# siyi-wind/MDViT

Measured on AMD Instinct MI355X. Metric: 512x512 images/sec MDViT train step (fwd+bwd, two-sweep, AdamW), higher is better.
Workload: dtype bf16x3 (fp32 storage; GEMM operands split hi+lo bf16, fp32 accumulate); 1 GPU; MDViT Sup+MLPFM train step, 4 domain(s) x bs=4 per GPU, 512x512, drop_rate=0.1 drop_path=0.1, bf16x3 GEMMs, data-parallel x1

## Files before the change

mdvit_amd/csrc/attn.hip:

```cpp
#include "common.h"
#include "conv_tile.h"

namespace {

constexpr int FA_T = 64;

struct FaGeom {
    int B, H, W, N, C, heads, Ch, s3, s5, s7;
    float scale;
};

typedef float fap_f32x16 __attribute__((ext_vector_type(16)));

template <int CH, bool SOFTMAX>
__global__ __launch_bounds__(256) void fa_partial_kernel(const float* __restrict__ X, long ldx, const float* __restrict__ Y, long ldy,
                                                         const float* __restrict__ ysc, float yscale,
                                                         float* __restrict__ ws_m, float* __restrict__ ws_s, float* __restrict__ ws_P,
                                                         FaGeom g, int NT, int NSUB,
                                                         const float* __restrict__ outp = nullptr, float* __restrict__ dU = nullptr, float* __restrict__ e_part = nullptr) {
    constexpr int GW = CH < 32 ? 32 : CH, NB = (GW + 31) / 32, GQ = GW / 4;
    constexpr int STAGE = 2 * FA_T * GW, RED = 4 * NB * 32 * NB * 32;
    __shared__ __attribute__((aligned(16))) float sm[(STAGE > RED ? STAGE : RED) + 3 * NB * 32 + (SOFTMAX ? 2 * 256 : 0)];
    float* xs = sm;
    float* ys = sm + FA_T * GW;
    float* s_m = sm + (STAGE > RED ? STAGE : RED);
    float* s_s = s_m + NB * 32;
    float* s_f = s_s + NB * 32;
    float* s_e = s_s;
    float* s_pm = s_f + NB * 32;
    float* s_ps = s_pm + 256;
    const int stile = blockIdx.x, c0 = blockIdx.y * GW, b = blockIdx.z;
    const int NTS = (NT + NSUB - 1) / NSUB;
    const int lane = threadIdx.x & 63, wave = threadIdx.x >> 6, l31 = lane & 31, lhi = lane >> 5;
    fap_f32x16 acc[NB][NB];
#pragma unroll
    for (int i = 0; i < NB; ++i)
#pragma unroll
        for (int j = 0; j < NB; ++j)
#pragma unroll
            for (int r = 0; r < 16; ++r) acc[i][j][r] = 0.f;
    if (SOFTMAX && threadIdx.x < NB * 32) { s_m[threadIdx.x] = -INFINITY; s_s[threadIdx.x] = 0.f; s_f[threadIdx.x] = 1.f; }
    if (SOFTMAX) s_ps[threadIdx.x] = 0.f;
    if (!SOFTMAX && e_part && threadIdx.x < NB * 32) s_e[threadIdx.x] = 0.f;
    constexpr int NVE = (FA_T * GQ + 255) / 256;
    float4 eacc[(!SOFTMAX) ? NVE : 1];
#pragma unroll
    for (int v = 0; v < ((!SOFTMAX) ? NVE : 1); ++v) eacc[v] = make_float4(0.f, 0.f, 0.f, 0.f);
    constexpr int NV = (FA_T * GQ + 255) / 256;
    float4 xv[NV], yv[NV], ov[(!SOFTMAX) ? NV : 1];
    auto request = [&](int tile) __attribute__((always_inline)) {
        const int n0r = min(tile, NT - 1) * FA_T;
#pragma unroll
        for (int v = 0; v < NV; ++v) {
            const int i = min((int)threadIdx.x + 256 * v, FA_T * GQ - 1), n = i / GQ, q = i % GQ;
            const long tok = (long)b * g.N + min(n0r + n, g.N - 1);
            xv[v] = *reinterpret_cast<const float4*>(X + tok * ldx + c0 + 4 * q);
            yv[v] = *reinterpret_cast<const float4*>(Y + tok * ldy + c0 + 4 * q);
            if (!SOFTMAX && e_part) ov[v] = *reinterpret_cast<const float4*>(outp + tok * (long)g.C + c0 + 4 * q);
        }
    };
    request(stile * NSUB);
    for (int sub = 0; sub < NSUB; ++sub) {
        const int tile = stile * NSUB + sub;
        if (tile >= NT) break;
        const int n0 = tile * FA_T, nt = min(FA_T, g.N - n0);
        {
#pragma unroll
            for (int v = 0; v < NV; ++v) {
                const int i = threadIdx.x + 256 * v, n = i / GQ;
                if (!(i < FA_T * GQ && n < nt)) {
                    xv[v] = make_float4(0.f, 0.f, 0.f, 0.f); yv[v] = xv[v];
                    if (!SOFTMAX) ov[v] = xv[v];
                }
            }
#pragma unroll
            for (int v = 0; v < NV; ++v) {
                const int i = threadIdx.x + 256 * v, n = i / GQ, q = i % GQ;
                if (i < FA_T * GQ) {
                    float4 y4 = yv[v];
                    if (!SOFTMAX) {
                        float4 sc = make_float4(yscale, yscale, yscale, yscale);
                        float4 a4 = make_float4(1.f, 1.f, 1.f, 1.f);
                        if (ysc) { a4 = *reinterpret_cast<const float4*>(ysc + (long)b * g.C + c0 + 4 * q); sc.x *= a4.x; sc.y *= a4.y; sc.z *= a4.z; sc.w *= a4.w; }
                        if (dU && n < nt)
                            *reinterpret_cast<float4*>(dU + ((long)b * g.N + n0 + n) * g.C + c0 + 4 * q) =
                                make_float4(a4.x * y4.x * xv[v].x, a4.y * y4.y * xv[v].y, a4.z * y4.z * xv[v].z, a4.w * y4.w * xv[v].w);
                        if (e_part) {
                            eacc[v].x = fmaf(y4.x, ov[v].x, eacc[v].x); eacc[v].y = fmaf(y4.y, ov[v].y, eacc[v].y);
                            eacc[v].z = fmaf(y4.z, ov[v].z, eacc[v].z); eacc[v].w = fmaf(y4.w, ov[v].w, eacc[v].w);
                        }
                        y4.x *= sc.x; y4.y *= sc.y; y4.z *= sc.z; y4.w *= sc.w;
                    }
                    *reinterpret_cast<float4*>(xs + n * GW + 4 * q) = xv[v];
                    *reinterpret_cast<float4*>(ys + n * GW + 4 * q) = y4;
                }
            }
        }
        if (sub + 1 < NSUB) request(tile + 1);
        __syncthreads();
        if (SOFTMAX) {
            constexpr int PER = 256 / GW;
            const int c = threadIdx.x % GW, sb = threadIdx.x / GW;
            const bool act = sb < PER;
            float m = -INFINITY;
            if (act)
                for (int n = sb; n < nt; n += PER) m = fmaxf(m, xs[n * GW + c]);
            if (act) s_pm[sb * GW + c] = m;
            __syncthreads();
            float m_old = 0.f, m_new = 0.f;
            if (act) {
                m_old = s_m[c];
                m_new = m_old;
#pragma unroll
                for (int j = 0; j < PER; ++j) m_new = fmaxf(m_new, s_pm[j * GW + c]);
                float ssum = 0.f;
                for (int n = sb; n < nt; n += PER) { const float e = expf(xs[n * GW + c] - m_new); xs[n * GW + c] = e; ssum += e; }
                for (int n = nt + sb; n < FA_T; n += PER) xs[n * GW + c] = 0.f;
                const float f = expf(m_old - m_new);
                s_ps[sb * GW + c] = fmaf(s_ps[sb * GW + c], f, ssum);
                if (sb == 0) s_f[c] = f;
            }
            __syncthreads();
            if (act && sb == 0) s_m[c] = m_new;
            if (sub > 0) {
#pragma unroll
                for (int i = 0; i < NB; ++i)
#pragma unroll
                    for (int q = 0; q < 4; ++q) {
                        const float4 f4 = *reinterpret_cast<const float4*>(s_f + 32 * i + 8 * q + 4 * lhi);
#pragma unroll
                        for (int j = 0; j < NB; ++j) {
                            acc[i][j][4 * q + 0] *= f4.x; acc[i][j][4 * q + 1] *= f4.y; acc[i][j][4 * q + 2] *= f4.z; acc[i][j][4 * q + 3] *= f4.w;
                        }
                    }
            }
        }
        constexpr int TPW = FA_T / 4;
#pragma unroll
        for (int kk = 0; kk < TPW / 2; ++kk) {
            const int n = wave * TPW + 2 * kk + lhi;
            float xa[NB], yb[NB];
#pragma unroll
            for (int i = 0; i < NB; ++i) { const int c = 32 * i + l31; xa[i] = c < GW ? xs[n * GW + c] : 0.f; }
#pragma unroll
            for (int j = 0; j < NB; ++j) { const int c = 32 * j + l31; yb[j] = c < GW ? ys[n * GW + c] : 0.f; }
#pragma unroll
            for (int i = 0; i < NB; ++i)
#pragma unroll
                for (int j = 0; j < NB; ++j) acc[i][j] = __builtin_amdgcn_mfma_f32_32x32x2f32(xa[i], yb[j], acc[i][j], 0, 0, 0);
        }
        __syncthreads();
    }
    if (SOFTMAX && threadIdx.x < GW) {
        const long o = ((long)b * NTS + stile) * g.C + c0 + threadIdx.x;
        float ssum = 0.f;
#pragma unroll
        for (int j = 0; j < 256 / GW; ++j) ssum += s_ps[j * GW + threadIdx.x];
        ws_m[o] = s_m[threadIdx.x]; ws_s[o] = ssum;
    }
    if (!SOFTMAX && e_part) {
#pragma unroll
        for (int v = 0; v < NVE; ++v) {
            const int i = threadIdx.x + 256 * v, q = i % GQ;
            if (i < FA_T * GQ) {
                atomicAdd(&s_e[4 * q + 0], eacc[v].x); atomicAdd(&s_e[4 * q + 1], eacc[v].y);
                atomicAdd(&s_e[4 * q + 2], eacc[v].z); atomicAdd(&s_e[4 * q + 3], eacc[v].w);
            }
        }
        __syncthreads();
        if (threadIdx.x < GW) e_part[((long)b * NTS + stile) * g.C + c0 + threadIdx.x] = s_e[threadIdx.x];
        __syncthreads();
    }
    constexpr int RW = NB * 32;
    float* red = sm + wave * RW * RW;
#pragma unroll
    for (int i = 0; i < NB; ++i)
#pragma unroll
        for (int j = 0; j < NB; ++j)
#pragma unroll
            for (int r = 0; r < 16; ++r) {
                const int c = 32 * i + 8 * (r >> 2) + 4 * lhi + (r & 3), e = 32 * j + l31;
                red[c * RW + e] = acc[i][j][r];
            }
    __syncthreads();
    for (int o = threadIdx.x; o < GW * CH; o += 256) {
        const int c = o / CH, el = o % CH, e = (c / CH) * CH + el;
        const float v = (sm[c * RW + e] + sm[RW * RW + c * RW + e]) + (sm[2 * RW * RW + c * RW + e] + sm[3 * RW * RW + c * RW + e]);
        ws_P[(((long)b * NTS + stile) * g.C + c0 + c) * CH + el] = v;
    }
}

template <int P> __device__ __forceinline__ float fa_dpp_quad_xor(float x) {
    constexpr int ctrl = P == 1 ? 0xB1 : (P == 2 ? 0x4E : 0x1B);
    return __builtin_bit_cast(float, __builtin_amdgcn_update_dpp(0, __builtin_bit_cast(int, x), ctrl, 0xF, 0xF, true));
}
template <int CH, bool SOFTMAX>
__global__ __launch_bounds__(256) __attribute__((amdgpu_waves_per_eu(2, 2))) void fa_partial_s8_kernel(const float* __restrict__ X, long ldx, const float* __restrict__ Y, long ldy,
                                                            const float* __restrict__ ysc, float yscale,
                                                            float* __restrict__ ws_m, float* __restrict__ ws_s, float* __restrict__ ws_P,
                                                            FaGeom g, int NT, int NSUB,
                                                            const float* __restrict__ outp, float* __restrict__ dU, float* __restrict__ e_part) {
    constexpr int C = 8 * CH, LPT = C / 4, SLOTS = 256 / LPT, LPH = CH / 4;
    constexpr int NACC = 4 * CH + 8;
    constexpr int GRP = (SOFTMAX && CH == 8) ? 4 : 2;
    extern __shared__ float fa_s_red[];
    const int stile = blockIdx.x, b = blockIdx.z;
    const int NTS = (NT + NSUB - 1) / NSUB;
    const int q = threadIdx.x % LPT, slot = threadIdx.x / LPT;
    const int c0 = 4 * q, hl = q % LPH;
    const int n_beg = stile * NSUB * FA_T, n_end = min(g.N, n_beg + NSUB * FA_T);
    float acc[4][CH];
#pragma unroll
    for (int j = 0; j < 4; ++j)
#pragma unroll
        for (int l = 0; l < CH; ++l) acc[j][l] = 0.f;
    float m[4] = {-INFINITY, -INFINITY, -INFINITY, -INFINITY}, ssum[4] = {0.f, 0.f, 0.f, 0.f}, eacc[4] = {0.f, 0.f, 0.f, 0.f};
    float sc[4] = {yscale, yscale, yscale, yscale}, av[4] = {1.f, 1.f, 1.f, 1.f};
    if (!SOFTMAX && ysc) {
        const float4 a4 = *reinterpret_cast<const float4*>(ysc + (long)b * C + c0);
        av[0] = a4.x; av[1] = a4.y; av[2] = a4.z; av[3] = a4.w;
#pragma unroll
        for (int j = 0; j < 4; ++j) sc[j] *= av[j];
    }
    struct Rows { float4 x[GRP], y[GRP], o[(!SOFTMAX) ? GRP : 1]; };
    auto request = [&](Rows& r, int n0) __attribute__((always_inline)) {
#pragma unroll
        for (int u = 0; u < GRP; ++u) {
            const long tok = (long)b * g.N + min(n0 + SLOTS * u, g.N - 1);
            r.x[u] = *reinterpret_cast<const float4*>(X + tok * ldx + c0);
            r.y[u] = *reinterpret_cast<const float4*>(Y + tok * ldy + c0);
            if (!SOFTMAX && e_part) r.o[u] = *reinterpret_cast<const float4*>(outp + tok * (long)C + c0);
        }
    };
    auto compute = [&](const Rows& r, int n0) __attribute__((always_inline)) {
        float xv[GRP][4], yv[GRP][4];
        bool ok[GRP];
#pragma unroll
        for (int u = 0; u < GRP; ++u) {
            ok[u] = n0 + SLOTS * u < n_end;
            xv[u][0] = r.x[u].x; xv[u][1] = r.x[u].y; xv[u][2] = r.x[u].z; xv[u][3] = r.x[u].w;
            yv[u][0] = r.y[u].x; yv[u][1] = r.y[u].y; yv[u][2] = r.y[u].z; yv[u][3] = r.y[u].w;
        }
        if (SOFTMAX) {
            float mn[4], f[4];
#pragma unroll
            for (int j = 0; j < 4; ++j) {
                mn[j] = m[j];
#pragma unroll
                for (int u = 0; u < GRP; ++u) mn[j] = fmaxf(mn[j], ok[u] ? xv[u][j] : -INFINITY);
                f[j] = (mn[j] == -INFINITY) ? 1.f : expf(m[j] - mn[j]);
                m[j] = mn[j];
                ssum[j] *= f[j];
#pragma unroll
                for (int l = 0; l < CH; ++l) acc[j][l] *= f[j];
            }
#pragma unroll
            for (int u = 0; u < GRP; ++u)
#pragma unroll
                for (int j = 0; j < 4; ++j) { xv[u][j] = ok[u] ? expf(xv[u][j] - mn[j]) : 0.f; ssum[j] += xv[u][j]; }
        }
#pragma unroll
        for (int u = 0; u < GRP; ++u) {
            float yh[CH];
            if (!SOFTMAX) {
                if (dU && ok[u]) {
                    const long tok = (long)b * g.N + n0 + SLOTS * u;
                    *reinterpret_cast<float4*>(dU + tok * C + c0) = make_float4(av[0] * yv[u][0] * xv[u][0], av[1] * yv[u][1] * xv[u][1], av[2] * yv[u][2] * xv[u][2], av[3] * yv[u][3] * xv[u][3]);
                }
                if (e_part && ok[u]) {
                    eacc[0] = fmaf(yv[u][0], r.o[u].x, eacc[0]); eacc[1] = fmaf(yv[u][1], r.o[u].y, eacc[1]);
                    eacc[2] = fmaf(yv[u][2], r.o[u].z, eacc[2]); eacc[3] = fmaf(yv[u][3], r.o[u].w, eacc[3]);
                }
#pragma unroll
                for (int j = 0; j < 4; ++j) { yh[j] = ok[u] ? yv[u][j] * sc[j] : 0.f; }
            } else {
#pragma unroll
                for (int j = 0; j < 4; ++j) yh[j] = yv[u][j];
            }
#pragma unroll
            for (int j = 0; j < 4; ++j) {
                yh[4 + j] = fa_dpp_quad_xor<1>(yh[j]);
                if (CH == 16) { yh[8 + j] = fa_dpp_quad_xor<2>(yh[j]); yh[12 + j] = fa_dpp_quad_xor<3>(yh[j]); }
            }
#pragma unroll
            for (int j = 0; j < 4; ++j)
#pragma unroll
                for (int l = 0; l < CH; ++l) acc[j][l] = fmaf(xv[u][j], yh[l], acc[j][l]);
        }
    };
    Rows ra, rb;
    int n = n_beg + slot;
    request(ra, n);
    for (; n < n_end; n += 2 * SLOTS * GRP) {
        request(rb, n + SLOTS * GRP);
        compute(ra, n);
        request(ra, n + 2 * SLOTS * GRP);
        compute(rb, n + SLOTS * GRP);
    }
    float* mine = fa_s_red + ((long)slot * LPT + q) * (NACC + 1);
#pragma unroll
    for (int j = 0; j < 4; ++j) {
#pragma unroll
        for (int l = 0; l < CH; ++l) mine[CH * j + l] = acc[j][l];
        mine[4 * CH + j] = SOFTMAX ? m[j] : eacc[j];
        mine[4 * CH + 4 + j] = ssum[j];
    }
    __syncthreads();
    if (threadIdx.x < C) {
        const int qq = threadIdx.x >> 2, j = threadIdx.x & 3, c = 4 * qq + j;
        const int hq = qq % LPH;
        float tot[CH], t1 = 0.f, mm = -INFINITY;
#pragma unroll
        for (int l = 0; l < CH; ++l) tot[l] = 0.f;
        if (SOFTMAX) {
            for (int sl = 0; sl < SLOTS; ++sl) mm = fmaxf(mm, fa_s_red[((long)sl * LPT + qq) * (NACC + 1) + 4 * CH + j]);
        }
        for (int sl = 0; sl < SLOTS; ++sl) {
            const float* r = fa_s_red + ((long)sl * LPT + qq) * (NACC + 1);
            float f = 1.f;
            if (SOFTMAX) { const float ms = r[4 * CH + j]; f = (ms == -INFINITY) ? 0.f : expf(ms - mm); t1 = fmaf(r[4 * CH + 4 + j], f, t1); }
            else t1 += r[4 * CH + j];
#pragma unroll
            for (int l = 0; l < CH; ++l) tot[l] = SOFTMAX ? fmaf(r[CH * j + l], f, tot[l]) : tot[l] + r[CH * j + l];
        }
        const long orow = ((long)b * NTS + stile) * C + c;
        float* P = ws_P + orow * CH;
#pragma unroll
        for (int l = 0; l < CH; ++l) P[4 * (hq ^ (l >> 2)) + (l & 3)] = tot[l];
        if (SOFTMAX) { ws_m[orow] = mm; ws_s[orow] = t1; }
        else if (e_part) e_part[orow] = t1;
    }
}
template <int CH, bool SOFTMAX>
static void fa_partial_stream_launch(dim3 grid, hipStream_t s, const float* X, long ldx, const float* Y, long ldy, const float* ysc, float yscale, float* ws_m, float* ws_s,
                                     float* ws_P, const FaGeom& g, int NT, int NSUB, const float* outp, float* dU, float* e_part) {
    constexpr int C = 8 * CH, LPT = C / 4, SLOTS = 256 / LPT;
    constexpr int smem = SLOTS * LPT * (4 * CH + 8 + 1) * (int)sizeof(float);
    static bool attr[64] = {false};
    int dev = 0;
    if (hipGetDevice(&dev) != hipSuccess || dev < 0 || dev >= 64) dev = 0;
    if (!attr[dev] && smem > 48 * 1024) {
// ... 473 lines not shown
        const float v = scale * (e[(long)b * C + c] - a[(long)b * C + c] * tot);
        dz[c] = v;
        dzbuf[(long)b * C + c] = v;
    }
    __syncthreads();
    float* tpart = sm + C;
    const int BD = blockDim.x;
    const int nseg = hid <= BD ? BD / hid : 1;
    for (int i0 = 0; i0 < hid; i0 += BD) {
        const int i = i0 + (int)threadIdx.x % (hid <= BD ? hid : BD), seg = hid <= BD ? (int)threadIdx.x / hid : 0;
        if (i < hid && seg < nseg) {
            const int c_beg = (int)((long)C * seg / nseg), c_end = (int)((long)C * (seg + 1) / nseg);
            float t = 0.f;
#pragma unroll 4
            for (int c = c_beg; c < c_end; ++c) t = fmaf(dz[c], W2[(long)c * hid + i], t);
            tpart[seg * hid + i] = t;
        }
    }
    __syncthreads();
    for (int i = threadIdx.x; i < hid; i += blockDim.x) {
        float s = 0.f;
        for (int d = 0; d < D; ++d) s = fmaf(label[(long)b * D + d], W1[(long)i * D + d], s);
        const float h = s + b1[i];
        float t = 0.f;
        for (int seg = 0; seg < nseg; ++seg) t += tpart[seg * hid + i];
        hbuf[(long)b * hid + i] = fmaxf(h, 0.f);
        dhbuf[(long)b * hid + i] = h > 0.f ? t : 0.f;
    }
}
__global__ __launch_bounds__(1024) void da_bwd_stage1_kernel(const float* __restrict__ label, const float* __restrict__ W1, const float* __restrict__ b1,
                                                            const float* __restrict__ W2, const float* __restrict__ a, const float* __restrict__ e,
                                                            float* __restrict__ dzbuf, float* __restrict__ hbuf, float* __restrict__ dhbuf,
                                                            int D, int hid, int C, int heads, float scale) {
    extern __shared__ float sm[];
    da_bwd_stage1_body(sm, label, W1, b1, W2, a, e, dzbuf, hbuf, dhbuf, D, hid, C, heads, scale);
}
__device__ __forceinline__ void da_bwd_stage2_body(const float* __restrict__ label, const float* __restrict__ dzbuf,
                                                   const float* __restrict__ hbuf, const float* __restrict__ dhbuf,
                                                   float* __restrict__ dW1, float* __restrict__ db1, float* __restrict__ dW2, float* __restrict__ db2,
                                                   int B, int D, int hid, int C) {
    const long i = (long)blockIdx.x * blockDim.x + threadIdx.x;
    const long nW2 = (long)C * hid, nW1 = (long)hid * D;
    if (i < nW2) {
        const int c = (int)(i / hid), j = (int)(i % hid);
        float s = 0.f;
        for (int b = 0; b < B; ++b) s = fmaf(dzbuf[(long)b * C + c], hbuf[(long)b * hid + j], s);
        dW2[i] = s;
    } else if (i < nW2 + nW1) {
        const long k = i - nW2;
        const int j = (int)(k / D), d = (int)(k % D);
        float s = 0.f;
        for (int b = 0; b < B; ++b) s = fmaf(dhbuf[(long)b * hid + j], label[(long)b * D + d], s);
        dW1[k] = s;
    } else if (i < nW2 + nW1 + C) {
        const int c = (int)(i - nW2 - nW1);
        float s = 0.f;
        for (int b = 0; b < B; ++b) s += dzbuf[(long)b * C + c];
        db2[c] = s;
    } else if (i < nW2 + nW1 + C + hid) {
        const int j = (int)(i - nW2 - nW1 - C);
        float s = 0.f;
        for (int b = 0; b < B; ++b) s += dhbuf[(long)b * hid + j];
        db1[j] = s;
    }
}
__global__ __launch_bounds__(256) void da_bwd_stage2_kernel(const float* __restrict__ label, const float* __restrict__ dzbuf,
                                                            const float* __restrict__ hbuf, const float* __restrict__ dhbuf,
                                                            float* __restrict__ dW1, float* __restrict__ db1, float* __restrict__ dW2, float* __restrict__ db2,
                                                            int B, int D, int hid, int C) {
    da_bwd_stage2_body(label, dzbuf, hbuf, dhbuf, dW1, db1, dW2, db2, B, D, hid, C);
}
__device__ __forceinline__ long da_many_ws_offset(const MdvitDaMany& m, int i, int B) {
    long off = 0;
    for (int j = 0; j < i; ++j) off += (long)B * m.C[j] + 2L * B * m.hid[j];
    return off;
}
__global__ __launch_bounds__(1024) void da_bwd_many_stage1_kernel(MdvitDaMany m, MdvitDaManyGrads g, const float* __restrict__ label, float* __restrict__ ws, int B, int D,
                                                                 float scale) {
    extern __shared__ float sm[];
    const int i = blockIdx.y;
    if (!g.e[i]) return;
    float* dzbuf = ws + da_many_ws_offset(m, i, B);
    float* hbuf = dzbuf + (long)B * m.C[i];
    float* dhbuf = hbuf + (long)B * m.hid[i];
    da_bwd_stage1_body(sm, label, m.W1[i], m.b1[i], m.W2[i], m.a[i], g.e[i], dzbuf, hbuf, dhbuf, D, m.hid[i], m.C[i], m.heads[i], scale);
}
__global__ __launch_bounds__(256) void da_bwd_many_stage2_kernel(MdvitDaMany m, MdvitDaManyGrads g, const float* __restrict__ label, const float* __restrict__ ws, int B, int D) {
    const int i = blockIdx.y;
    const int hid = m.hid[i], C = m.C[i];
    if (!g.e[i] || (long)blockIdx.x * blockDim.x >= (long)C * hid + (long)hid * D + C + hid) return;
    const float* dzbuf = ws + da_many_ws_offset(m, i, B);
    const float* hbuf = dzbuf + (long)B * C;
    const float* dhbuf = hbuf + (long)B * hid;
    da_bwd_stage2_body(label, dzbuf, hbuf, dhbuf, g.dW1[i], g.db1[i], g.dW2[i], g.db2[i], B, D, hid, C);
}

bool make_geom(FaGeom& g, int B, int H, int W, int C, int heads, int s3, int s5, int s7) {
    if (B <= 0 || H <= 0 || W <= 0 || C <= 0 || heads <= 0 || C % heads != 0 || C % 4 != 0) return false;
    if (s3 + s5 + s7 != heads) return false;
    g.B = B; g.H = H; g.W = W; g.N = H * W; g.C = C; g.heads = heads; g.Ch = C / heads; g.s3 = s3; g.s5 = s5; g.s7 = s7;
    g.scale = 1.0f / sqrtf((float)g.Ch);
    return true;
}

size_t fa_ws_floats(int B, int N, int C, int heads) {
    const int Ch = C / heads;
    const long NT = (N + FA_T - 1) / FA_T;
    const long fwd = (long)B * NT * C * (2 + Ch);
    const long wg_rows = (long)(cdiv(C, 32) + 2) * B > 1024 ? (long)(cdiv(C, 32) + 2) * B : 1024;
    const long part = wg_rows * 32 * 50 > 1024L * B * C ? wg_rows * 32 * 50 : 1024L * B * C;
    const long bwd = 2L * B * N * C + (long)B * C * (1 + Ch) + (long)B * NT * C * Ch + part;
    return (size_t)(fwd > bwd ? fwd : bwd);
}

int fa_nsub(int NT) { return NT >= 128 ? 8 : (NT >= 64 ? 4 : (NT >= 16 ? 2 : 1)); }

bool fa_built(const FaGeom& g) { return ((g.Ch == 8 || g.Ch == 16) && g.heads == 8) || ((g.Ch == 40 || g.Ch == 64) && g.C <= 512); }
#define FA_CHECK_BUILT(fn, g) MDVIT_CHECK_ARG(fa_built(g), MDVIT_E_SHAPE, fn ": C=%d with %d heads (head dim %d) not built: built are 8 heads at C = 64 / 128 (head dim 8 / 16) " \
                                              "and head dim 40 / 64 with C <= 512 (8 heads at C = 320 / 512)", (g).C, (g).heads, (g).Ch)

int quad_grid(long work_quads, int QC, int max_blocks) {
    int a = QC, b = 256;
    while (b) { int t = a % b; a = b; b = t; }
    const int gmul = QC / a;
    long want = (work_quads + 256L * 4 - 1) / (256L * 4);
    if (want > max_blocks) want = max_blocks;
    if (want < 1) want = 1;
    return (int)((want + gmul - 1) / gmul * gmul);
}

}

extern "C" size_t mdvit_factoratt_ws_bytes(int32_t B, int32_t N, int32_t C, int32_t heads) {
    if (B <= 0 || N <= 0 || C <= 0 || heads <= 0 || C % heads) return 0;
    return fa_ws_floats(B, N, C, heads) * sizeof(float);
}

extern "C" int mdvit_factoratt_fwd(const float* qkv, const float* w3, const float* b3, const float* w5, const float* b5,
                                   const float* w7, const float* b7, const float* a, float* out, float* U, float* kmax, float* ksum, float* Mmat,
                                   void* ws, size_t ws_bytes, int32_t B, int32_t H, int32_t W, int32_t C, int32_t heads,
                                   int32_t s3, int32_t s5, int32_t s7, void* stream) {
    hipStream_t s = (hipStream_t)stream;
    FaGeom g;
    MDVIT_CHECK_ARG(make_geom(g, B, H, W, C, heads, s3, s5, s7), MDVIT_E_SHAPE, "factoratt_fwd: bad geometry B=%d H=%d W=%d C=%d heads=%d splits=%d/%d/%d", B, H, W, C, heads, s3, s5, s7);
    FA_CHECK_BUILT("factoratt_fwd", g);
    MDVIT_CHECK_ARG(ws_bytes >= fa_ws_floats(B, g.N, C, heads) * sizeof(float), MDVIT_E_WORKSPACE, "factoratt_fwd: workspace too small (%zu bytes)", ws_bytes);
    const int Ch = g.Ch, NT0 = cdiv(g.N, FA_T);
    const int NSUB = fa_nsub(NT0);
    const int NT = cdiv(NT0, NSUB);
    float* ws_m = (float*)ws;
    float* ws_s = ws_m + (long)B * NT * C;
    float* ws_P = ws_s + (long)B * NT * C;
#define FA_PART_STREAM(CHV) fa_partial_stream_launch<CHV, true>(dim3(NT, 1, B), s, qkv + C, (long)3 * C, qkv + 2 * C, (long)3 * C, nullptr, 1.f, ws_m, ws_s, ws_P, g, NT0, NSUB, nullptr, nullptr, nullptr)
#define FA_PART_TILES(CHV) hipLaunchKernelGGL((fa_partial_kernel<CHV, true>), dim3(NT, C / CHV, B), dim3(256), 0, s, \
                       qkv + C, (long)3 * C, qkv + 2 * C, (long)3 * C, (const float*)nullptr, 1.f, ws_m, ws_s, ws_P, g, NT0, NSUB)
    switch (Ch) {
        case 8: FA_PART_STREAM(8); break;
        case 16: FA_PART_STREAM(16); break;
        case 40: FA_PART_TILES(40); break;
        case 64: FA_PART_TILES(64); break;
    }
#undef FA_PART_STREAM
#undef FA_PART_TILES
    if (NT > 8)
        hipLaunchKernelGGL((fa_combine_softmax_kernel<32>), dim3(cdiv((long)C * g.Ch, 8), B), dim3(256), 0, s, ws_m, ws_s, ws_P, kmax, ksum, Mmat, g, NT);
    else if (NT > 2)
        hipLaunchKernelGGL((fa_combine_softmax_kernel<4>), dim3(cdiv((long)C * g.Ch, 64), B), dim3(256), 0, s, ws_m, ws_s, ws_P, kmax, ksum, Mmat, g, NT);
    else
        hipLaunchKernelGGL((fa_combine_softmax_kernel<1>), dim3(cdiv((long)C * g.Ch, 256), B), dim3(256), 0, s, ws_m, ws_s, ws_P, kmax, ksum, Mmat, g, NT);
    const int c5 = s3 * Ch, c7 = (s3 + s5) * Ch;
    const CtGeom cg{B, g.H, g.W};
    {
        const int xoff[3] = {2 * C, 2 * C + c5, 2 * C + c7}, yoff[3] = {0, c5, c7}, ncls[3] = {s3 * Ch, s5 * Ch, s7 * Ch};
        const float* const ws3[3] = {w3, w5, w7};
        const float* const bs3[3] = {b3, b5, b7};
        launch_conv3<false>(qkv, 3L * C, xoff, ws3, bs3, U, (long)C, yoff, cg, ncls, s);
    }
    {
        const int TLN = max(1, 256 / C), block = TLN * C;
        int tpb = TLN * 32;
        while (tpb > TLN * 8 && (long)cdiv(g.N, tpb) * B < 1024) tpb /= 2;
        while ((long)cdiv(g.N, tpb) * B > 8192) tpb *= 2;
        dim3 grid(cdiv(g.N, tpb), B);
#define FA_OUT_LAUNCH(CHV) hipLaunchKernelGGL((fa_out_kernel<CHV>), grid, dim3(block), sizeof(float) * FA_OUT_U * TLN * C, s, qkv, U, Mmat, a, out, g, TLN, tpb)
        switch (Ch) {
            case 8: FA_OUT_LAUNCH(8); break;
            case 16: FA_OUT_LAUNCH(16); break;
            case 40: FA_OUT_LAUNCH(40); break;
            case 64: FA_OUT_LAUNCH(64); break;
        }
#undef FA_OUT_LAUNCH
    }
    MDVIT_LAUNCH_CHECK();
    return MDVIT_OK;
}

extern "C" int mdvit_factoratt_bwd(const float* dout, const float* qkv, const float* out, const float* U,
                                   const float* w3, const float* b3, const float* w5, const float* b5, const float* w7, const float* b7,
                                   const float* a, const float* kmax, const float* ksum, const float* Mmat,
                                   float* dqkv, float* e, float* dw3, float* db3, float* dw5, float* db5, float* dw7, float* db7,
                                   void* ws, size_t ws_bytes, int32_t B, int32_t H, int32_t W, int32_t C, int32_t heads,
                                   int32_t s3, int32_t s5, int32_t s7, void* stream) {
    hipStream_t s = (hipStream_t)stream;
    FaGeom g;
    MDVIT_CHECK_ARG(make_geom(g, B, H, W, C, heads, s3, s5, s7), MDVIT_E_SHAPE, "factoratt_bwd: bad geometry B=%d H=%d W=%d C=%d heads=%d", B, H, W, C, heads);
    FA_CHECK_BUILT("factoratt_bwd", g);
    MDVIT_CHECK_ARG(ws_bytes >= fa_ws_floats(B, g.N, C, heads) * sizeof(float), MDVIT_E_WORKSPACE, "factoratt_bwd: workspace too small (%zu bytes)", ws_bytes);
    MDVIT_CHECK_ARG((a == nullptr) == (e == nullptr), MDVIT_E_SHAPE, "factoratt_bwd: a and e must both be given or both be NULL");
    const int Ch = g.Ch, NT = cdiv(g.N, FA_T);
    float* dU = (float*)ws;
    float* dVc = dU + (long)B * g.N * C;
    float* tcol = dVc + (long)B * g.N * C;
    float* dM = tcol + (long)B * C;
    float* ws_P = dM + (long)B * C * Ch;
    const bool want_wgrad = dw3 != nullptr;
    MDVIT_CHECK_ARG(want_wgrad ? (db3 && dw5 && db5 && dw7 && db7) : !(db3 || dw5 || db5 || dw7 || db7), MDVIT_E_SHAPE,
                    "factoratt_bwd: the six crpe gradient outputs must be all given or all NULL");
    if (dqkv == nullptr) {
        MDVIT_CHECK_ARG(e != nullptr && !want_wgrad, MDVIT_E_SHAPE, "factoratt_bwd: dqkv == NULL asks for e alone");
        const int QC0 = C / 4;
        const int gx = quad_grid((long)g.N * QC0, QC0, 512);
        float* e_part = ws_P + (long)B * NT * C * Ch;
        hipLaunchKernelGGL(fa_bwd_prep_kernel, dim3(gx, B), dim3(256), sizeof(float) * C, s, dout, qkv, out, a, (float*)nullptr, e_part, g);
        MDVIT_LAUNCH_CHECK();
        return mdvit_reduce_partials_batched(e_part, B, gx, C, e, s);
    }
    const int NSUBb = fa_nsub(NT), NTS = cdiv(NT, NSUBb);
    float* e_part = ws_P + (long)B * NT * C * Ch;
#define FA_PART_STREAM(CHV) fa_partial_stream_launch<CHV, false>(dim3(NTS, 1, B), s, qkv, (long)3 * C, dout, (long)C, a, g.scale, nullptr, nullptr, ws_P, g, NT, NSUBb, out, dU, e ? e_part : nullptr)
#define FA_PART_TILES(CHV) hipLaunchKernelGGL((fa_partial_kernel<CHV, false>), dim3(NTS, C / CHV, B), dim3(256), 0, s, \
                       qkv, (long)3 * C, dout, (long)C, a, g.scale, (float*)nullptr, (float*)nullptr, ws_P, g, NT, NSUBb, out, dU, e ? e_part : (float*)nullptr)
    switch (Ch) {
        case 8: FA_PART_STREAM(8); break;
        case 16: FA_PART_STREAM(16); break;
        case 40: FA_PART_TILES(40); break;
        case 64: FA_PART_TILES(64); break;
    }
#undef FA_PART_STREAM
#undef FA_PART_TILES
    if (e) {
        const int rc = mdvit_reduce_partials_batched(e_part, B, NTS, C, e, s);
        if (rc != MDVIT_OK) return rc;
    }
    const int c5 = s3 * Ch, c7 = (s3 + s5) * Ch;
    const CtGeom cg{B, g.H, g.W};
    if (want_wgrad) {
        float* wg_part = ws_P + (long)B * NT * C * Ch;
        const int goff[3] = {0, c5, c7}, xoff3[3] = {2 * C, 2 * C + c5, 2 * C + c7}, ncls3[3] = {s3 * Ch, s5 * Ch, s7 * Ch};
        float* const dws[3] = {dw3, dw5, dw7};
        float* const dbs[3] = {db3, db5, db7};
        launch_conv3_wgrad(dU, (long)C, goff, qkv, 3L * C, xoff3, dws, dbs, wg_part, cg, ncls3, s, 0);
    }
    {
        const int off[3] = {0, c5, c7}, ncls[3] = {s3 * Ch, s5 * Ch, s7 * Ch};
        const float* const ws3[3] = {w3, w5, w7};
        launch_conv3<true>(dU, (long)C, off, ws3, nullptr, dVc, (long)C, off, cg, ncls, s);
    }
    if (Ch >= 32) {
        const int ntiles = cdiv(g.N, 32);
        int tpb = 8;
        while (tpb > 2 && (long)cdiv(ntiles, tpb) * heads * B < 256) tpb /= 2;
        const int gx = cdiv(ntiles, tpb);
        const long nwg = (long)gx * heads * B;
        const int xcd_map = nwg % 8 == 0 && nwg < (1L << 30);
        dim3 grid = xcd_map ? dim3((unsigned)nwg, 1, 1) : dim3(gx, heads, B);
        if (Ch == 40) hipLaunchKernelGGL((fa_bwd_apply3_kernel<40>), grid, dim3(384), 0, s, dout, qkv, U, dVc, Mmat, a, kmax, ksum, ws_P, NTS, dqkv, g, tpb, gx, xcd_map);
        else hipLaunchKernelGGL((fa_bwd_apply3_kernel<64>), grid, dim3(384), 0, s, dout, qkv, U, dVc, Mmat, a, kmax, ksum, ws_P, NTS, dqkv, g, tpb, gx, xcd_map);
    } else {
        int tpbk = Ch == 8 ? 1024 : 512;
        while (tpbk > 128 && (long)cdiv(g.N, tpbk) * B < 512) tpbk /= 2;
        const dim3 grid(cdiv(g.N, tpbk), B);
        if (Ch == 8) hipLaunchKernelGGL(fa_bwd_apply_tab_kernel<8>, grid, dim3(256), 0, s, dout, qkv, U, dVc, Mmat, a, kmax, ksum, ws_P, NTS, dqkv, g, tpbk);
        else hipLaunchKernelGGL(fa_bwd_apply_tab_kernel<16>, grid, dim3(256), 0, s, dout, qkv, U, dVc, Mmat, a, kmax, ksum, ws_P, NTS, dqkv, g, tpbk);
    }
    MDVIT_LAUNCH_CHECK();
    return MDVIT_OK;
}

extern "C" int mdvit_factoratt_wgrad(const float* qkv, void* ws, size_t ws_bytes, float* dw3, float* db3, float* dw5, float* db5,
                                     float* dw7, float* db7, int32_t B, int32_t H, int32_t W, int32_t C, int32_t heads,
                                     int32_t s3, int32_t s5, int32_t s7, int32_t accumulate, void* stream) {
    hipStream_t s = (hipStream_t)stream;
    FaGeom g;
    MDVIT_CHECK_ARG(make_geom(g, B, H, W, C, heads, s3, s5, s7), MDVIT_E_SHAPE, "factoratt_wgrad: bad geometry");
    MDVIT_CHECK_ARG(ws_bytes >= fa_ws_floats(B, g.N, C, heads) * sizeof(float), MDVIT_E_WORKSPACE, "factoratt_wgrad: workspace too small");
    MDVIT_CHECK_ARG(dw3 && db3 && dw5 && db5 && dw7 && db7, MDVIT_E_SHAPE, "factoratt_wgrad: all six outputs are required");
    const int Ch = g.Ch, NT = cdiv(g.N, FA_T);
    const float* dU = (const float*)ws;
    float* wg_part = (float*)ws + 2L * B * g.N * C + (long)B * C * (1 + Ch) + (long)B * NT * C * Ch;
    const int c5 = s3 * Ch, c7 = (s3 + s5) * Ch;
    const CtGeom cg{B, g.H, g.W};
    const int goff[3] = {0, c5, c7}, xoff3[3] = {2 * C, 2 * C + c5, 2 * C + c7}, ncls3[3] = {s3 * Ch, s5 * Ch, s7 * Ch};
    float* const dws[3] = {dw3, dw5, dw7};
    float* const dbs[3] = {db3, db5, db7};
    launch_conv3_wgrad(dU, (long)C, goff, qkv, 3L * C, xoff3, dws, dbs, wg_part, cg, ncls3, s, accumulate);
    MDVIT_LAUNCH_CHECK();
    return MDVIT_OK;
}

extern "C" int mdvit_da_fwd(const float* label, const float* W1, const float* b1, const float* W2, const float* b2, float* a,
                            int32_t B, int32_t D, int32_t hid, int32_t C, int32_t heads, void* stream) {
    MDVIT_CHECK_ARG(B > 0 && D > 0 && hid > 0 && C > 0 && heads > 0 && C % heads == 0, MDVIT_E_SHAPE, "da_fwd: bad shape");
    const int G = max(1, min(1024 / C, hid));
    hipLaunchKernelGGL(da_fwd_kernel, dim3(B), dim3(1024), sizeof(float) * (hid + C + (size_t)(G + 1) * C), (hipStream_t)stream, label, W1, b1, W2, b2, a, D, hid, C, heads);
    MDVIT_LAUNCH_CHECK();
    return MDVIT_OK;
}

extern "C" int mdvit_da_fwd_many(const MdvitDaMany* m, const float* label, int32_t B, int32_t D, void* stream) {
    MDVIT_CHECK_ARG(m && label && B > 0 && D > 0 && m->n > 0 && m->n <= MDVIT_DA_MANY_MAX, MDVIT_E_SHAPE, "da_fwd_many: bad arguments");
    size_t smem = 0;
    for (int i = 0; i < m->n; ++i) {
        const int C = m->C[i], hid = m->hid[i];
        MDVIT_CHECK_ARG(m->W1[i] && m->b1[i] && m->W2[i] && m->b2[i] && m->a[i] && hid > 0 && C > 0 && m->heads[i] > 0 && C % m->heads[i] == 0, MDVIT_E_SHAPE,
                        "da_fwd_many: bad adapter %d", i);
        const int G = max(1, min(1024 / C, hid));
        smem = std::max(smem, sizeof(float) * (hid + C + (size_t)(G + 1) * C));
    }
    MDVIT_CHECK_ARG(smem <= 64 * 1024, MDVIT_E_SHAPE, "da_fwd_many: an adapter needs %zu bytes of LDS", smem);
    hipLaunchKernelGGL(da_fwd_many_kernel, dim3(B, m->n), dim3(1024), smem, (hipStream_t)stream, *m, label, D);
    MDVIT_LAUNCH_CHECK();
    return MDVIT_OK;
}

extern "C" size_t mdvit_da_ws_bytes(int32_t B, int32_t hid, int32_t C) {
    if (B <= 0 || hid <= 0 || C <= 0) return 0;
    return sizeof(float) * ((size_t)B * C + 2 * (size_t)B * hid);
}

extern "C" size_t mdvit_da_many_ws_bytes(const MdvitDaMany* m, int32_t B) {
    if (!m || m->n <= 0 || m->n > MDVIT_DA_MANY_MAX || B <= 0) return 0;
    size_t t = 0;
    for (int i = 0; i < m->n; ++i) t += mdvit_da_ws_bytes(B, m->hid[i], m->C[i]);
    return t;
}

extern "C" int mdvit_da_bwd_many(const MdvitDaMany* m, const MdvitDaManyGrads* g, const float* label, float scale, void* ws, size_t ws_bytes, int32_t B, int32_t D,
                                 void* stream) {
    MDVIT_CHECK_ARG(m && g && m->n > 0 && m->n <= MDVIT_DA_MANY_MAX && B > 0 && D > 0, MDVIT_E_SHAPE, "da_bwd_many: bad shape");
    MDVIT_CHECK_ARG(ws_bytes >= mdvit_da_many_ws_bytes(m, B), MDVIT_E_WORKSPACE, "da_bwd_many: workspace too small");
    size_t smem = 0;
    long most = 0;
    bool any = false;
    for (int i = 0; i < m->n; ++i) {
        MDVIT_CHECK_ARG(m->hid[i] > 0 && m->C[i] > 0 && m->heads[i] > 0 && m->C[i] % m->heads[i] == 0, MDVIT_E_SHAPE, "da_bwd_many: bad adapter shape");
        if (!g->e[i]) continue;
        MDVIT_CHECK_ARG(g->dW1[i] && g->db1[i] && g->dW2[i] && g->db2[i], MDVIT_E_SHAPE, "da_bwd_many: an adapter with e needs its four gradient outputs");
        any = true;
        smem = max(smem, sizeof(float) * (m->C[i] + (size_t)max(m->hid[i], 1024)));
        most = max(most, (long)m->C[i] * m->hid[i] + (long)m->hid[i] * D + m->C[i] + m->hid[i]);
    }
    if (!any) return MDVIT_OK;
    hipStream_t s = (hipStream_t)stream;
    hipLaunchKernelGGL(da_bwd_many_stage1_kernel, dim3(B, m->n), dim3(1024), smem, s, *m, *g, label, (float*)ws, B, D, scale);
    hipLaunchKernelGGL(da_bwd_many_stage2_kernel, dim3(cdiv(most, 256), m->n), dim3(256), 0, s, *m, *g, label, (const float*)ws, B, D);
    MDVIT_LAUNCH_CHECK();
    return MDVIT_OK;
}

extern "C" int mdvit_da_bwd(const float* label, const float* W1, const float* b1, const float* W2, const float* b2, const float* a,
                            const float* e, float scale, float* dW1, float* db1, float* dW2, float* db2, void* ws, size_t ws_bytes,
                            int32_t B, int32_t D, int32_t hid, int32_t C, int32_t heads, void* stream) {
    hipStream_t s = (hipStream_t)stream;
    (void)b2;
    MDVIT_CHECK_ARG(B > 0 && D > 0 && hid > 0 && C > 0 && heads > 0 && C % heads == 0, MDVIT_E_SHAPE, "da_bwd: bad shape");
    MDVIT_CHECK_ARG(ws_bytes >= mdvit_da_ws_bytes(B, hid, C), MDVIT_E_WORKSPACE, "da_bwd: workspace too small");
    float* dzbuf = (float*)ws;
    float* hbuf = dzbuf + (long)B * C;
    float* dhbuf = hbuf + (long)B * hid;
    hipLaunchKernelGGL(da_bwd_stage1_kernel, dim3(B), dim3(1024), sizeof(float) * (C + (size_t)max(hid, 1024)), s, label, W1, b1, W2, a, e, dzbuf, hbuf, dhbuf, D, hid, C, heads, scale);
    const long total = (long)C * hid + (long)hid * D + C + hid;
    hipLaunchKernelGGL(da_bwd_stage2_kernel, dim3(cdiv(total, 256)), dim3(256), 0, s, label, dzbuf, hbuf, dhbuf, dW1, db1, dW2, db2, B, D, hid, C);
    MDVIT_LAUNCH_CHECK();
    return MDVIT_OK;
}
```

Measured before the change: 517.1 images/s.

## Rewrite factor-attention partial kernel to process four heads per block, one per wave

Replaces the tiled partial kernel for head dims 40 and 64 with a wide variant where each block covers four heads and each wave computes one head's Ch x Ch product with 16x16x4 MFMAs. The online softmax max and sum now live in registers and use wave shuffles, which removes several per-tile barriers and the cross-wave LDS reduction of the accumulators. LDS rows are padded to avoid bank conflicts, and occupancy is pinned to two waves per EU. Risks include more register pressure, smaller 32-token tiles, and a smaller grid along the channel axis.

```diff
diff --git a/mdvit_amd/csrc/attn.hip b/mdvit_amd/csrc/attn.hip
--- a/mdvit_amd/csrc/attn.hip
+++ b/mdvit_amd/csrc/attn.hip
@@ -10,183 +10,158 @@
     float scale;
 };
 
-typedef float fap_f32x16 __attribute__((ext_vector_type(16)));
-
+typedef float faw_f32x4 __attribute__((ext_vector_type(4)));
+constexpr int FAW_T = 32;
+constexpr int FAW_HW = 4;
 template <int CH, bool SOFTMAX>
-__global__ __launch_bounds__(256) void fa_partial_kernel(const float* __restrict__ X, long ldx, const float* __restrict__ Y, long ldy,
-                                                         const float* __restrict__ ysc, float yscale,
-                                                         float* __restrict__ ws_m, float* __restrict__ ws_s, float* __restrict__ ws_P,
-                                                         FaGeom g, int NT, int NSUB,
-                                                         const float* __restrict__ outp = nullptr, float* __restrict__ dU = nullptr, float* __restrict__ e_part = nullptr) {
-    constexpr int GW = CH < 32 ? 32 : CH, NB = (GW + 31) / 32, GQ = GW / 4;
-    constexpr int STAGE = 2 * FA_T * GW, RED = 4 * NB * 32 * NB * 32;
-    __shared__ __attribute__((aligned(16))) float sm[(STAGE > RED ? STAGE : RED) + 3 * NB * 32 + (SOFTMAX ? 2 * 256 : 0)];
+__global__ __launch_bounds__(256) __attribute__((amdgpu_waves_per_eu(2, 2))) void fa_partial_wide_kernel(const float* __restrict__ X, long ldx, const float* __restrict__ Y, long ldy,
+                                                              const float* __restrict__ ysc, float yscale,
+                                                              float* __restrict__ ws_m, float* __restrict__ ws_s, float* __restrict__ ws_P,
+                                                              FaGeom g, int NT, int NSUB,
+                                                              const float* __restrict__ outp, float* __restrict__ dU, float* __restrict__ e_part) {
+    constexpr int GWW = FAW_HW * CH, GQ = GWW / 4, NBK = (CH + 15) / 16, KK = FAW_T / 4;
+    constexpr int LDW = GWW + 16;
+    constexpr int NV = FAW_T * GQ / 256;
+    constexpr int NVE = (256 % GQ == 0) ? 1 : NV;
+    static_assert(CH % 4 == 0 && (FAW_T * GQ) % 256 == 0 && LDW % 64 != 0 && LDW % 32 != 0, "staging / bank layout");
+    static_assert(NVE * 256 * 4 <= 2 * FAW_T * LDW, "the e slots meet in the operand tiles' LDS");
+    __shared__ __attribute__((aligned(16))) float sm[2 * FAW_T * LDW + GWW];
     float* xs = sm;
-    float* ys = sm + FA_T * GW;
-    float* s_m = sm + (STAGE > RED ? STAGE : RED);
-    float* s_s = s_m + NB * 32;
-    float* s_f = s_s + NB * 32;
-    float* s_e = s_s;
-    float* s_pm = s_f + NB * 32;
-    float* s_ps = s_pm + 256;
-    const int stile = blockIdx.x, c0 = blockIdx.y * GW, b = blockIdx.z;
+    float* ys = sm + FAW_T * LDW;
+    float* s_a = ys + FAW_T * LDW;
+    const int stile = blockIdx.x, c0 = blockIdx.y * GWW, b = blockIdx.z;
     const int NTS = (NT + NSUB - 1) / NSUB;
-    const int lane = threadIdx.x & 63, wave = threadIdx.x >> 6, l31 = lane & 31, lhi = lane >> 5;
-    fap_f32x16 acc[NB][NB];
-#pragma unroll
-    for (int i = 0; i < NB; ++i)
-#pragma unroll
-        for (int j = 0; j < NB; ++j)
-#pragma unroll
-            for (int r = 0; r < 16; ++r) acc[i][j][r] = 0.f;
-    if (SOFTMAX && threadIdx.x < NB * 32) { s_m[threadIdx.x] = -INFINITY; s_s[threadIdx.x] = 0.f; s_f[threadIdx.x] = 1.f; }
-    if (SOFTMAX) s_ps[threadIdx.x] = 0.f;
-    if (!SOFTMAX && e_part && threadIdx.x < NB * 32) s_e[threadIdx.x] = 0.f;
-    constexpr int NVE = (FA_T * GQ + 255) / 256;
+    const int lane = threadIdx.x & 63, wave = threadIdx.x >> 6, l16 = lane & 15, lg = lane >> 4;
+    const int n_beg = stile * NSUB * FA_T, n_end = min(g.N, n_beg + NSUB * FA_T);
+    const bool head_ok = c0 + (wave + 1) * CH <= g.C;
+    if (!SOFTMAX) {
+        for (int i = threadIdx.x; i < GWW; i += 256) s_a[i] = (ysc && c0 + i < g.C) ? ysc[(long)b * g.C + c0 + i] : 1.f;
+        __syncthreads();
+    }
+    faw_f32x4 acc[NBK][NBK];
+#pragma unroll
+    for (int i = 0; i < NBK; ++i)
+#pragma unroll
+        for (int j = 0; j < NBK; ++j) acc[i][j] = faw_f32x4{0.f, 0.f, 0.f, 0.f};
+    float m_run[NBK], s_run[NBK];
+    int cj[NBK];
+#pragma unroll
+    for (int j = 0; j < NBK; ++j) { m_run[j] = -INFINITY; s_run[j] = 0.f; cj[j] = min(16 * j + l16, CH - 1); }
     float4 eacc[(!SOFTMAX) ? NVE : 1];
 #pragma unroll
     for (int v = 0; v < ((!SOFTMAX) ? NVE : 1); ++v) eacc[v] = make_float4(0.f, 0.f, 0.f, 0.f);
-    constexpr int NV = (FA_T * GQ + 255) / 256;
     float4 xv[NV], yv[NV], ov[(!SOFTMAX) ? NV : 1];
-    auto request = [&](int tile) __attribute__((always_inline)) {
-        const int n0r = min(tile, NT - 1) * FA_T;
+    auto request = [&](int n0) __attribute__((always_inline)) {
 #pragma unroll
         for (int v = 0; v < NV; ++v) {
-            const int i = min((int)threadIdx.x + 256 * v, FA_T * GQ - 1), n = i / GQ, q = i % GQ;
-            const long tok = (long)b * g.N + min(n0r + n, g.N - 1);
-            xv[v] = *reinterpret_cast<const float4*>(X + tok * ldx + c0 + 4 * q);
-            yv[v] = *reinterpret_cast<const float4*>(Y + tok * ldy + c0 + 4 * q);
-            if (!SOFTMAX && e_part) ov[v] = *reinterpret_cast<const float4*>(outp + tok * (long)g.C + c0 + 4 * q);
+            const int i = (int)threadIdx.x + 256 * v, n = i / GQ, q = i % GQ;
+            const long tok = (long)b * g.N + min(n0 + n, g.N - 1);
+            const int cq = c0 + 4 * q < g.C ? c0 + 4 * q : c0;
+            xv[v] = *reinterpret_cast<const float4*>(X + tok * ldx + cq);
+            yv[v] = *reinterpret_cast<const float4*>(Y + tok * ldy + cq);
+            if (!SOFTMAX && e_part) ov[v] = *reinterpret_cast<const float4*>(outp + tok * (long)g.C + cq);
         }
     };
-    request(stile * NSUB);
-    for (int sub = 0; sub < NSUB; ++sub) {
-        const int tile = stile * NSUB + sub;
-        if (tile >= NT) break;
-        const int n0 = tile * FA_T, nt = min(FA_T, g.N - n0);
-        {
-#pragma unroll
-            for (int v = 0; v < NV; ++v) {
-                const int i = threadIdx.x + 256 * v, n = i / GQ;
-                if (!(i < FA_T * GQ && n < nt)) {
-                    xv[v] = make_float4(0.f, 0.f, 0.f, 0.f); yv[v] = xv[v];
-                    if (!SOFTMAX) ov[v] = xv[v];
+    request(n_beg);
+    for (int n0 = n_beg; n0 < n_end; n0 += FAW_T) {
+        const int nt = min(FAW_T, n_end - n0);
+#pragma unroll
+        for (int v = 0; v < NV; ++v) {
+            const int i = (int)threadIdx.x + 256 * v, n = i / GQ, q = i % GQ;
+            const bool valid = n < nt && c0 + 4 * q < g.C;
+            const float xpad = SOFTMAX ? -INFINITY : 0.f;
+            float4 x4 = valid ? xv[v] : make_float4(xpad, xpad, xpad, xpad);
+            float4 y4 = valid ? yv[v] : make_float4(0.f, 0.f, 0.f, 0.f);
+            if (!SOFTMAX) {
+                const float4 a4 = *reinterpret_cast<const float4*>(s_a + 4 * q);
+                float4 sc = make_float4(yscale, yscale, yscale, yscale);
+                sc.x *= a4.x; sc.y *= a4.y; sc.z *= a4.z; sc.w *= a4.w;
+                if (dU && valid)
+                    *reinterpret_cast<float4*>(dU + ((long)b * g.N + n0 + n) * g.C + c0 + 4 * q) =
+                        make_float4(a4.x * y4.x * x4.x, a4.y * y4.y * x4.y, a4.z * y4.z * x4.z, a4.w * y4.w * x4.w);
+                if (e_part) {
+                    const float4 o4 = valid ? ov[v] : make_float4(0.f, 0.f, 0.f, 0.f);
+                    float4& ea = eacc[NVE == 1 ? 0 : v];
+                    ea.x = fmaf(y4.x, o4.x, ea.x); ea.y = fmaf(y4.y, o4.y, ea.y); ea.z = fmaf(y4.z, o4.z, ea.z); ea.w = fmaf(y4.w, o4.w, ea.w);
                 }
-            }
-#pragma unroll
-            for (int v = 0; v < NV; ++v) {
-                const int i = threadIdx.x + 256 * v, n = i / GQ, q = i % GQ;
-                if (i < FA_T * GQ) {
-                    float4 y4 = yv[v];
-                    if (!SOFTMAX) {
-                        float4 sc = make_float4(yscale, yscale, yscale, yscale);
-                        float4 a4 = make_float4(1.f, 1.f, 1.f, 1.f);
-                        if (ysc) { a4 = *reinterpret_cast<const float4*>(ysc + (long)b * g.C + c0 + 4 * q); sc.x *= a4.x; sc.y *= a4.y; sc.z *= a4.z; sc.w *= a4.w; }
-                        if (dU && n < nt)
-                            *reinterpret_cast<float4*>(dU + ((long)b * g.N + n0 + n) * g.C + c0 + 4 * q) =
-                                make_float4(a4.x * y4.x * xv[v].x, a4.y * y4.y * xv[v].y, a4.z * y4.z * xv[v].z, a4.w * y4.w * xv[v].w);
-                        if (e_part) {
-                            eacc[v].x = fmaf(y4.x, ov[v].x, eacc[v].x); eacc[v].y = fmaf(y4.y, ov[v].y, eacc[v].y);
-                            eacc[v].z = fmaf(y4.z, ov[v].z, eacc[v].z); eacc[v].w = fmaf(y4.w, ov[v].w, eacc[v].w);
-                        }
-                        y4.x *= sc.x; y4.y *= sc.y; y4.z *= sc.z; y4.w *= sc.w;
-                    }
-                    *reinterpret_cast<float4*>(xs + n * GW + 4 * q) = xv[v];
-                    *reinterpret_cast<float4*>(ys + n * GW + 4 * q) = y4;
+                y4.x *= sc.x; y4.y *= sc.y; y4.z *= sc.z; y4.w *= sc.w;
+            }
+            *reinterpret_cast<float4*>(xs + n * LDW + 4 * q) = x4;
+            *reinterpret_cast<float4*>(ys + n * LDW + 4 * q) = y4;
+        }
+        if (n0 + FAW_T < n_end) request(n0 + FAW_T);
+        __syncthreads();
+        if (head_ok) {
+            const float* xh = xs + lg * LDW + wave * CH;
+            const float* yh = ys + lg * LDW + wave * CH;
+            float xb[NBK][KK];
+#pragma unroll
+            for (int j = 0; j < NBK; ++j)
+#pragma unroll
+                for (int kk = 0; kk < KK; ++kk) xb[j][kk] = xh[4 * kk * LDW + cj[j]];
+            if (SOFTMAX) {
+#pragma unroll
+                for (int j = 0; j < NBK; ++j) {
+                    float tm = xb[j][0];
+#pragma unroll
+                    for (int kk = 1; kk < KK; ++kk) tm = fmaxf(tm, xb[j][kk]);
+                    tm = fmaxf(tm, __shfl_xor(tm, 16));
+                    tm = fmaxf(tm, __shfl_xor(tm, 32));
+                    const float m_new = fmaxf(m_run[j], tm);
+                    const float f = expf(m_run[j] - m_new);
+                    m_run[j] = m_new;
+                    float ts = 0.f;
+#pragma unroll
+                    for (int kk = 0; kk < KK; ++kk) { xb[j][kk] = expf(xb[j][kk] - m_new); ts += xb[j][kk]; }
+                    s_run[j] = fmaf(s_run[j], f, ts);
+#pragma unroll
+                    for (int i = 0; i < NBK; ++i) { acc[i][j][0] *= f; acc[i][j][1] *= f; acc[i][j][2] *= f; acc[i][j][3] *= f; }
                 }
             }
-        }
-        if (sub + 1 < NSUB) request(tile + 1);
+#pragma unroll
+            for (int kk = 0; kk < KK; ++kk) {
+                float ya[NBK];
+#pragma unroll
+                for (int i = 0; i < NBK; ++i) ya[i] = yh[4 * kk * LDW + cj[i]];
+#pragma unroll
+                for (int i = 0; i < NBK; ++i)
+#pragma unroll
+                    for (int j = 0; j < NBK; ++j) acc[i][j] = __builtin_amdgcn_mfma_f32_16x16x4f32(ya[i], xb[j][kk], acc[i][j], 0, 0, 0);
+            }
+        }
         __syncthreads();
-        if (SOFTMAX) {
-            constexpr int PER = 256 / GW;
-            const int c = threadIdx.x % GW, sb = threadIdx.x / GW;
-            const bool act = sb < PER;
-            float m = -INFINITY;
-            if (act)
-                for (int n = sb; n < nt; n += PER) m = fmaxf(m, xs[n * GW + c]);
-            if (act) s_pm[sb * GW + c] = m;
-            __syncthreads();
-            float m_old = 0.f, m_new = 0.f;
-            if (act) {
-                m_old = s_m[c];
-                m_new = m_old;
-#pragma unroll
-                for (int j = 0; j < PER; ++j) m_new = fmaxf(m_new, s_pm[j * GW + c]);
-                float ssum = 0.f;
-                for (int n = sb; n < nt; n += PER) { const float e = expf(xs[n * GW + c] - m_new); xs[n * GW + c] = e; ssum += e; }
-                for (int n = nt + sb; n < FA_T; n += PER) xs[n * GW + c] = 0.f;
-                const float f = expf(m_old - m_new);
-                s_ps[sb * GW + c] = fmaf(s_ps[sb * GW + c], f, ssum);
-                if (sb == 0) s_f[c] = f;
-            }
-            __syncthreads();
-            if (act && sb == 0) s_m[c] = m_new;
-            if (sub > 0) {
-#pragma unroll
-                for (int i = 0; i < NB; ++i)
-#pragma unroll
-                    for (int q = 0; q < 4; ++q) {
-                        const float4 f4 = *reinterpret_cast<const float4*>(s_f + 32 * i + 8 * q + 4 * lhi);
-#pragma unroll
-                        for (int j = 0; j < NB; ++j) {
-                            acc[i][j][4 * q + 0] *= f4.x; acc[i][j][4 * q + 1] *= f4.y; acc[i][j][4 * q + 2] *= f4.z; acc[i][j][4 * q + 3] *= f4.w;
-                        }
-                    }
-            }
-        }
-        constexpr int TPW = FA_T / 4;
-#pragma unroll
-        for (int kk = 0; kk < TPW / 2; ++kk) {
-            const int n = wave * TPW + 2 * kk + lhi;
-            float xa[NB], yb[NB];
-#pragma unroll
-            for (int i = 0; i < NB; ++i) { const int c = 32 * i + l31; xa[i] = c < GW ? xs[n * GW + c] : 0.f; }
-#pragma unroll
-            for (int j = 0; j < NB; ++j) { const int c = 32 * j + l31; yb[j] = c < GW ? ys[n * GW + c] : 0.f; }
-#pragma unroll
-            for (int i = 0; i < NB; ++i)
-#pragma unroll
-                for (int j = 0; j < NB; ++j) acc[i][j] = __builtin_amdgcn_mfma_f32_32x32x2f32(xa[i], yb[j], acc[i][j], 0, 0, 0);
-        }
+    }
+    if (head_ok) {
+        const long row = ((long)b * NTS + stile) * g.C + c0 + wave * CH;
+#pragma unroll
+        for (int j = 0; j < NBK; ++j) {
+            const int c = 16 * j + l16;
+            if (SOFTMAX) {
+                float s = s_run[j];
+                s += __shfl_xor(s, 16);
+                s += __shfl_xor(s, 32);
+                if (lg == 0 && c < CH) { ws_m[row + c] = m_run[j]; ws_s[row + c] = s; }
+            }
+            if (c < CH) {
+#pragma unroll
+                for (int i = 0; i < NBK; ++i) {
+                    const int e0 = 16 * i + 4 * lg;
+                    if (e0 < CH) *reinterpret_cast<float4*>(ws_P + (row + c) * CH + e0) = make_float4(acc[i][j][0], acc[i][j][1], acc[i][j][2], acc[i][j][3]);
+                }
+            }
+        }
+    }
+    if (!SOFTMAX && e_part) {
+        float4* et = reinterpret_cast<float4*>(sm);
+#pragma unroll
+        for (int v = 0; v < NVE; ++v) et[threadIdx.x + 256 * v] = eacc[v];
         __syncthreads();
-    }
-    if (SOFTMAX && threadIdx.x < GW) {
-        const long o = ((long)b * NTS + stile) * g.C + c0 + threadIdx.x;
-        float ssum = 0.f;
-#pragma unroll
-        for (int j = 0; j < 256 / GW; ++j) ssum += s_ps[j * GW + threadIdx.x];
-        ws_m[o] = s_m[threadIdx.x]; ws_s[o] = ssum;
-    }
-    if (!SOFTMAX && e_part) {
-#pragma unroll
-        for (int v = 0; v < NVE; ++v) {
-            const int i = threadIdx.x + 256 * v, q = i % GQ;
-            if (i < FA_T * GQ) {
-                atomicAdd(&s_e[4 * q + 0], eacc[v].x); atomicAdd(&s_e[4 * q + 1], eacc[v].y);
-                atomicAdd(&s_e[4 * q + 2], eacc[v].z); atomicAdd(&s_e[4 * q + 3], eacc[v].w);
-            }
-        }
-        __syncthreads();
-        if (threadIdx.x < GW) e_part[((long)b * NTS + stile) * g.C + c0 + threadIdx.x] = s_e[threadIdx.x];
-        __syncthreads();
-    }
-    constexpr int RW = NB * 32;
-    float* red = sm + wave * RW * RW;
-#pragma unroll
-    for (int i = 0; i < NB; ++i)
-#pragma unroll
-        for (int j = 0; j < NB; ++j)
-#pragma unroll
-            for (int r = 0; r < 16; ++r) {
-                const int c = 32 * i + 8 * (r >> 2) + 4 * lhi + (r & 3), e = 32 * j + l31;
-                red[c * RW + e] = acc[i][j][r];
-            }
-    __syncthreads();
-    for (int o = threadIdx.x; o < GW * CH; o += 256) {
-        const int c = o / CH, el = o % CH, e = (c / CH) * CH + el;
-        const float v = (sm[c * RW + e] + sm[RW * RW + c * RW + e]) + (sm[2 * RW * RW + c * RW + e] + sm[3 * RW * RW + c * RW + e]);
-        ws_P[(((long)b * NTS + stile) * g.C + c0 + c) * CH + el] = v;
+        if (threadIdx.x < GWW && c0 + (int)threadIdx.x < g.C) {
+            const int q = threadIdx.x >> 2, j = threadIdx.x & 3;
+            float s = 0.f;
+            for (int n = 0; n < NVE * 256 / GQ; ++n) s += reinterpret_cast<const float*>(et + n * GQ + q)[j];
+            e_part[((long)b * NTS + stile) * g.C + c0 + threadIdx.x] = s;
+        }
     }
 }
 
@@ -966,8 +941,9 @@
     float* ws_s = ws_m + (long)B * NT * C;
     float* ws_P = ws_s + (long)B * NT * C;
 #define FA_PART_STREAM(CHV) fa_partial_stream_launch<CHV, true>(dim3(NT, 1, B), s, qkv + C, (long)3 * C, qkv + 2 * C, (long)3 * C, nullptr, 1.f, ws_m, ws_s, ws_P, g, NT0, NSUB, nullptr, nullptr, nullptr)
-#define FA_PART_TILES(CHV) hipLaunchKernelGGL((fa_partial_kernel<CHV, true>), dim3(NT, C / CHV, B), dim3(256), 0, s, \
-                       qkv + C, (long)3 * C, qkv + 2 * C, (long)3 * C, (const float*)nullptr, 1.f, ws_m, ws_s, ws_P, g, NT0, NSUB)
+#define FA_PART_TILES(CHV) hipLaunchKernelGGL((fa_partial_wide_kernel<CHV, true>), dim3(NT, cdiv(heads, FAW_HW), B), dim3(256), 0, s, \
+                       qkv + C, (long)3 * C, qkv + 2 * C, (long)3 * C, (const float*)nullptr, 1.f, ws_m, ws_s, ws_P, g, NT0, NSUB, \
+                       (const float*)nullptr, (float*)nullptr, (float*)nullptr)
     switch (Ch) {
         case 8: FA_PART_STREAM(8); break;
         case 16: FA_PART_STREAM(16); break;
@@ -1042,7 +1018,7 @@
     const int NSUBb = fa_nsub(NT), NTS = cdiv(NT, NSUBb);
     float* e_part = ws_P + (long)B * NT * C * Ch;
 #define FA_PART_STREAM(CHV) fa_partial_stream_launch<CHV, false>(dim3(NTS, 1, B), s, qkv, (long)3 * C, dout, (long)C, a, g.scale, nullptr, nullptr, ws_P, g, NT, NSUBb, out, dU, e ? e_part : nullptr)
-#define FA_PART_TILES(CHV) hipLaunchKernelGGL((fa_partial_kernel<CHV, false>), dim3(NTS, C / CHV, B), dim3(256), 0, s, \
+#define FA_PART_TILES(CHV) hipLaunchKernelGGL((fa_partial_wide_kernel<CHV, false>), dim3(NTS, cdiv(heads, FAW_HW), B), dim3(256), 0, s, \
                        qkv, (long)3 * C, dout, (long)C, a, g.scale, (float*)nullptr, (float*)nullptr, ws_P, g, NT, NSUBb, out, dU, e ? e_part : (float*)nullptr)
     switch (Ch) {
         case 8: FA_PART_STREAM(8); break;
```

New measurement: 520.1 images/s, median of 6. About the same (+0.6%).
